# RaulAstudillo06/BOCF

Hardware: AMD Instinct MI355X
Metric: acquisition evals/sec (candidates x MC-samples/sec), uEI_noiseless batch call; GP-fit ms alongside (higher is better)
Workload: dtype f64; 1 GPU; BASELINE configs[2]: m=4 rbf-ARD GP, N=4096 d=8, S=1024 MC samples, C=65536 candidates, noise 1e-06, top-16 selection; N=4096, d=8, m=4, S=1024, C=65536, rccl_ranks_seen=0

## Files before the change

bocf_amd/_ffi.py:

```python
import contextlib
import ctypes
import os

import numpy as np

HERE = os.path.dirname(os.path.abspath(__file__))
LIB_PATH = os.path.join(HERE, "lib", "libbocf_hip.so")
PROBES_LIB_PATH = os.path.join(HERE, "lib", "libbocf_hip_probes.so")

KERN_RBF, KERN_SE, KERN_MATERN52, KERN_MATERN32 = 0, 1, 2, 3
ADD_NOISE, CLIP = 1, 2
ACQ_EI, ACQ_PI = 0, 1
UTIL_LINEAR, UTIL_NEG_SQ_DIST, UTIL_NEG_SUM_EXP, UTIL_NEG_EXP_COS, UTIL_ROSENBROCK = 0, 1, 2, 3, 4
UTIL_PROGRAM = 5
EU_MEAN, EU_CLOSED, EU_MC = 0, 1, 2
EU_MODES = {"mean": EU_MEAN, "closed": EU_CLOSED, "mc": EU_MC}


def eu_mode(mode):
    return EU_MODES[mode] if isinstance(mode, str) else int(mode)


_c_double_p = ctypes.POINTER(ctypes.c_double)
_c_ll_p = ctypes.POINTER(ctypes.c_longlong)
_ctx_p = ctypes.c_void_p

FDF_CALLBACK = ctypes.CFUNCTYPE(ctypes.c_int, ctypes.c_void_p, _c_double_p, ctypes.POINTER(ctypes.c_int), ctypes.c_int, ctypes.c_int, _c_double_p, _c_double_p)

SIGNATURES = {
    "bocf_version": (ctypes.c_int, []),
    "bocf_last_error": (ctypes.c_char_p, []),
    "bocf_create": (ctypes.c_int, [ctypes.c_int, ctypes.POINTER(_ctx_p)]),
    "bocf_destroy": (None, [_ctx_p]),
    "bocf_set_option": (ctypes.c_int, [_ctx_p, ctypes.c_char_p, ctypes.c_longlong]),
    "bocf_fit": (ctypes.c_int, [_ctx_p, _c_double_p, _c_double_p, ctypes.c_int, ctypes.c_int, ctypes.c_int, ctypes.c_int,
                                _c_double_p, _c_double_p, _c_double_p, ctypes.c_int, _c_double_p, _c_double_p]),
    "bocf_set_kernel_ids": (ctypes.c_int, [_ctx_p, ctypes.POINTER(ctypes.c_int), ctypes.c_int]),
    "bocf_update_targets": (ctypes.c_int, [_ctx_p, _c_double_p, _c_double_p]),
    "bocf_append": (ctypes.c_int, [_ctx_p, _c_double_p, _c_double_p, _c_double_p]),
    "bocf_lml_gradients": (ctypes.c_int, [_ctx_p, _c_double_p, _c_double_p, _c_double_p]),
    "bocf_infer": (ctypes.c_int, [_ctx_p, _c_double_p, _c_double_p, ctypes.c_int, ctypes.c_int, ctypes.c_int, ctypes.c_int, _c_double_p,
                                  _c_double_p, _c_double_p, ctypes.c_int, _c_double_p, _c_double_p, _c_double_p, _c_double_p, _c_double_p]),
    "bocf_last_fit_info": (ctypes.c_int, [_ctx_p, ctypes.POINTER(ctypes.c_int), ctypes.c_int]),
    "bocf_hmc": (ctypes.c_int, [_ctx_p, _c_double_p, _c_double_p, ctypes.c_int, ctypes.c_int, ctypes.c_int, ctypes.c_int, _c_double_p, ctypes.c_int,
                                ctypes.POINTER(ctypes.c_int), ctypes.c_double, ctypes.c_double, _c_double_p, _c_double_p, ctypes.c_int, ctypes.c_int,
                                ctypes.c_double, ctypes.c_int, ctypes.c_int, _c_double_p, ctypes.POINTER(ctypes.c_int), ctypes.POINTER(ctypes.c_int),
                                ctypes.POINTER(ctypes.c_int), _c_ll_p]),
    "bocf_hmc_streamed": (ctypes.c_int, [_ctx_p, _c_double_p, _c_double_p, ctypes.c_int, ctypes.c_int, ctypes.c_int, ctypes.c_int, _c_double_p, ctypes.c_int,
                                         ctypes.POINTER(ctypes.c_int), ctypes.c_double, ctypes.c_double, _c_double_p, _c_double_p, ctypes.c_int, ctypes.c_int,
                                         ctypes.c_double, _c_double_p, ctypes.POINTER(ctypes.c_int), ctypes.POINTER(ctypes.c_int),
                                         ctypes.POINTER(ctypes.c_int), _c_ll_p]),
    "bocf_get_factor": (ctypes.c_int, [_ctx_p, ctypes.c_int, _c_double_p, _c_double_p]),
    "bocf_get_train_kernel": (ctypes.c_int, [_ctx_p, ctypes.c_int, _c_double_p]),
    "bocf_set_posterior": (ctypes.c_int, [_ctx_p, ctypes.c_int, ctypes.c_int, ctypes.c_int, _c_double_p, _c_double_p, _c_double_p]),
    "bocf_set_candidates": (ctypes.c_int, [_ctx_p, _c_double_p, ctypes.c_int]),
    "bocf_predict": (ctypes.c_int, [_ctx_p, ctypes.c_int, _c_double_p, _c_double_p]),
    "bocf_predict_cov_column": (ctypes.c_int, [_ctx_p, ctypes.c_int, _c_double_p]),
    "bocf_predict_gradients": (ctypes.c_int, [_ctx_p, _c_double_p, _c_double_p]),
    "bocf_posterior_cov": (ctypes.c_int, [_ctx_p, _c_double_p, ctypes.c_int, _c_double_p, ctypes.c_int, ctypes.c_int, _c_double_p]),
    "bocf_posterior_samples": (ctypes.c_int, [_ctx_p, ctypes.c_int, _c_double_p, ctypes.c_int, ctypes.c_int, _c_double_p, _c_double_p]),
    "bocf_thompson_select": (ctypes.c_int, [_ctx_p, ctypes.c_int, _c_double_p, ctypes.c_int, _c_double_p, ctypes.c_int, ctypes.c_int, _c_ll_p,
                                            _c_double_p]),
    "bocf_set_ref_points": (ctypes.c_int, [_ctx_p, _c_double_p, ctypes.c_int]),
    "bocf_cov_to_ref": (ctypes.c_int, [_ctx_p, ctypes.c_int, _c_double_p, _c_double_p]),
    "bocf_conditioned_variance": (ctypes.c_int, [_ctx_p, ctypes.c_int, ctypes.c_int, _c_double_p, _c_double_p]),
    "bocf_acq_kg": (ctypes.c_int, [_ctx_p, ctypes.c_int, ctypes.c_int, _c_double_p, ctypes.c_int, _c_double_p, ctypes.c_int, _c_double_p, ctypes.c_int,
                                   _c_double_p, ctypes.c_int, _c_double_p, _c_double_p]),
# ... 133 lines not shown
```

bocf_amd/csrc/acq.hip:

```cpp
#include "bocf_internal.h"
#include <type_traits>
#include <cstdlib>
#include "../../include/bocf_hip.h"
#include "utility_dev.h"

__global__ __launch_bounds__(256) void best_so_far_kernel(const double* __restrict__ mu_train, int N, int m, int util_kind,
                                                          const double* __restrict__ theta, int theta_dim,
                                                          const double* __restrict__ params, double* __restrict__ best) {
  const int l = blockIdx.x;
  const double* th = theta + (long)l * theta_dim;
  double mx = -INFINITY;
  for (int i = threadIdx.x; i < N; i += 256) {
    double y[BOCF_MAX_M];
#pragma unroll
    for (int j = 0; j < BOCF_MAX_M; ++j) y[j] = j < m ? mu_train[(long)j * N + i] : 0.0;
    const double v = utility_eval(util_kind, th, params, y, m);
    mx = fmax(mx, v);
  }
  __shared__ double red[256];
  red[threadIdx.x] = mx;
  __syncthreads();
  for (int o = 128; o > 0; o >>= 1) {
    if (threadIdx.x < o) red[threadIdx.x] = fmax(red[threadIdx.x], red[threadIdx.x + o]);
    __syncthreads();
// ... 65 lines not shown
  double acq = 0.0;
  for (int l = 0; l < a.L; ++l) {
    const double* th = a.theta + (long)l * a.theta_dim;
    const double best = a.kind == BOCF_ACQ_EI ? a.best[l] : a.best[l] + 1e-6;
    double part = 0.0;
    for (int s = lane; s < a.S; s += 64) {
      double y[BOCF_MAX_M];
#pragma unroll
      for (int j = 0; j < BOCF_MAX_M; ++j) y[j] = j < a.m ? mu[j] + sg[j] * a.Wt[(long)j * a.S + s] : 0.0;
      const double v = utility_eval(a.util_kind, th, a.util_params, y, a.m);
      if (a.kind == BOCF_ACQ_EI) part += fmax(v - best, 0.0);
      else part += (v - best) > 0.0 ? 1.0 : 0.0;
    }
#pragma unroll
    for (int o = 32; o > 0; o >>= 1) part += __shfl_xor(part, o, 64);
    acq += (part / (double)a.S) * a.prob[l];
  }
  if (lane == 0) a.acq[c] = (a.accumulate ? a.acq[c] : 0.0) + acq * a.scale;
}

template <int M>
__global__ __launch_bounds__(256) void acq_mc_m_kernel(AcqArgs a) {
  const int lane = threadIdx.x & 63;
  const int c = blockIdx.x * 4 + (threadIdx.x >> 6);
  if (c >= a.C) return;
  double mu[M], sg[M];
#pragma unroll
  for (int j = 0; j < M; ++j) {
    mu[j] = a.mean[(long)j * a.ld + c];
    sg[j] = sqrt(a.var[(long)j * a.ld + c]);
  }
  double acq = 0.0;
  for (int l = 0; l < a.L; ++l) {
    const double* th = a.theta + (long)l * a.theta_dim;
    const double best = a.kind == BOCF_ACQ_EI ? a.best[l] : a.best[l] + 1e-6;
    double part = 0.0;
    for (int s = lane; s < a.S; s += 64) {
      double y[BOCF_MAX_M];
#pragma unroll
      for (int j = 0; j < BOCF_MAX_M; ++j) y[j] = 0.0;
#pragma unroll
      for (int j = 0; j < M; ++j) y[j] = mu[j] + sg[j] * a.Wt[(long)j * a.S + s];
      const double v = utility_eval(a.util_kind, th, a.util_params, y, M);
      if (a.kind == BOCF_ACQ_EI) part += fmax(v - best, 0.0);
      else part += (v - best) > 0.0 ? 1.0 : 0.0;
    }
#pragma unroll
    for (int o = 32; o > 0; o >>= 1) part += __shfl_xor(part, o, 64);
    acq += (part / (double)a.S) * a.prob[l];
  }
  if (lane == 0) a.acq[c] = (a.accumulate ? a.acq[c] : 0.0) + acq * a.scale;
}

void launch_acq_mc(const AcqArgs& a, hipStream_t s) {
  if (a.C == 0) return;
  if (a.util_kind == BOCF_UTIL_PROGRAM) {
    launch_acq_mc_prog(a, s);
    return;
  }
  const dim3 grid((unsigned)((a.C + 3) / 4));
  if (a.m >= 1 && a.m <= 8) {
#define LM(M) case M: BOCF_LAUNCH((acq_mc_m_kernel<M>), grid, dim3(256), 0, s, a); break;
    switch (a.m) { LM(1) LM(2) LM(3) LM(4) LM(5) LM(6) LM(7) LM(8) default: break; }
#undef LM
    return;
  }
  BOCF_LAUNCH(acq_mc_kernel, grid, dim3(256), 0, s, a);
}

__global__ __launch_bounds__(256) void acq_linear_grad_kernel(AcqArgs a) {
  const int c = blockIdx.x * 256 + threadIdx.x;
  if (c >= a.C) return;
  double mean[BOCF_MAX_M], var[BOCF_MAX_M];
#pragma unroll
  for (int j = 0; j < BOCF_MAX_M; ++j) {
    mean[j] = j < a.m ? a.mean[(long)j * a.ld + c] : 0.0;
    var[j] = j < a.m ? a.var[(long)j * a.ld + c] : 0.0;
  }
  double acq = 0.0;
  if (!a.accumulate)
    for (int q = 0; q < a.d; ++q) a.dacq[(long)c * a.d + q] = 0.0;
  for (int l = 0; l < a.L; ++l) {
    const double* th = a.theta + (long)l * a.theta_dim;
    double mu = 0.0, s2 = 0.0;
#pragma unroll
    for (int j = 0; j < BOCF_MAX_M; ++j)
      if (j < a.m) {
        mu += th[j] * mean[j];
        s2 += (th[j] * th[j]) * var[j];
      }
    const double sigma = sqrt(s2);
    double Phi, phi, u, val;
    if (a.kind == BOCF_ACQ_EI) {
      u = (mu - a.best[l]) / sigma;
      Phi = 0.5 * erfc(-u / 1.41421356237309504880);
      phi = exp(-0.5 * u * u) / 2.50662827463100050242;
      val = (mu - a.best[l]) * Phi + sigma * phi;
    } else {
      const double sfl = sigma < 1e-10 ? 1e-10 : sigma;
      u = (mu - (a.best[l] + 1e-6)) / sfl;
      Phi = 0.5 * erfc(-u / 1.41421356237309504880);
      phi = exp(-0.5 * u * u) / 2.50662827463100050242;
      val = Phi;
    }
    acq += val * a.prob[l];
    for (int q = 0; q < a.d; ++q) {
      double dmu = 0.0, dv = 0.0;
#pragma unroll
      for (int j = 0; j < BOCF_MAX_M; ++j)
        if (j < a.m) {
// ... 307 lines not shown
```

bocf_amd/csrc/bocf_ctx.h:

```cpp
#pragma once
#include "bocf_internal.h"
#include "chol_plan.h"
#include "predict_plan.h"
#include "../../include/bocf_hip.h"

#include <map>
#include <string>
#include <utility>
#include <vector>

int bocf_fail(const char* what, const char* detail);
void bocf_set_error(const char* text);
int bocf_launch_status();
int bocf_plan_cholesky(bocf_ctx* c, bool kinv, CholPlan* out);
int bocf_run_cholesky(bocf_ctx* c, const CholPlan& plan, bool counters_zeroed = false);
int bocf_run_trtri(bocf_ctx* c, bool early_done);
int bocf_comm_broadcast(bocf_ctx* c, double* buf, size_t count, int root);
int bocf_comm_group(bool start);
int bocf_comm_abort(bocf_ctx* c);
int bocf_comm_allreduce_sum(bocf_ctx* c, double* buf, size_t count);
#define fail bocf_fail
#define HIPCHK(expr)                                                         \
  do {                                                                       \
    hipError_t e_ = (expr);                                                  \
// ... 71 lines not shown
  long long fits_done = 0;
  int last_schedule = 0;
  int sched_m = 0;
  int force_sched_timeout = 0;
  int data_N = 0, data_d = 0, data_m = 0;
  int fused_infer = 1;
  int reuse_data = 0;
  int skip_mu_train = 0;
  DevBuf gpart, gout;
  DevBuf hmc_buf;
  double* infer_out = nullptr;
  size_t infer_out_cap = 0;
  bool fitted = false;
  bool canned = false;
  int N = 0, Np = 0, d = 0, m = 0, kernel_id = 0;
  long xs_stride = 0;
  std::vector<int> kernel_ids;
  std::vector<int> pending_ids;
  std::vector<KernHyp> hyp;
  std::vector<double> jitter;
  std::vector<int> last_info;
  DevBuf R32;
  bool r32_valid = false;
  int predict_f32 = 0;
  DevBuf Ri8, Ri8e, Ki8, Ki8e;
  bool ri8_valid = false;
  int predict_i8 = 0, i8_group = 0;
  DevBuf X, Xs, S, R, RT, E, ET, T, yc, tvec, rvec, dvec, alpha, lml, jit, hypd, info, mu_train;
  int C = 0;
  DevBuf Xc;
  long chunk = 65536;
  long workspace_mb = 24576;
  DevBuf Kstar, meanpart, sumsq, mean, var, acq, Vbuf, dmean, dvar, dacq, Vs, Ws;
  int pred_cap = 0;
  DevBuf theta, prob, best, params, Wt;
  std::vector<double> last_params;
  long long mu_epoch = 0;
  long long best_epoch = -1; int best_sig = -1;
  int S_mc = 0;
  bool have_acq = false;
  DevBuf prog_buf;
  UtilProg prog;
  DevBuf blk_idx, blk_val, out_idx, out_val;
  DevBuf eu_theta, eu_rows, eu_Z, eu_val, eu_grad;
  int eu_S = 0, eu_L = 0, eu_m = 0;
  void* eu_pin = nullptr;
  size_t eu_pin_cap = 0;
  hipEvent_t ev_eu_pin = nullptr;
  bool profile = false;
  double test_diag_shift = 0.0;
  int prefetch1 = 0;
  int kstar_valu_probe = 0;
  int small_path = 1;
  int hyper_samples = 1;
  int acq_hyper_samples = 0;
  int best_group = -1;
  int swizzle = -1;
  std::vector<std::pair<hipEvent_t, hipEvent_t>> events;
  double prof_flops = 0.0;
  std::map<std::string, std::vector<std::pair<hipEvent_t, hipEvent_t>>> phases;
  int shard_fit = 0;
  int shard_fit_simulate = 0;
  bool sharded = false;
  bocf_ctx* shard_helper = nullptr;
  DevBuf shard_meta;
  void* comm = nullptr;
  int world = 1, rank = 0;
  DevBuf pack, gidx, gval;
  bocf_ctx* ts_helper = nullptr;
  DevBuf ts_X, ts_K, ts_V, ts_mp, ts_mu, ts_Z, ts_jit, ts_u, ts_theta, ts_params, ts_out;
  std::vector<DevBuf> ts_F;
  std::vector<int> ts_S;
  int kg_na = 0;
  DevBuf kg_XA, kg_VA, kg_Wa, kg_muA, kg_s2A, kg_nug;
  DevBuf kg_V, kg_W, kg_cov, kg_s2c, kg_dcov, kg_dmean, kg_dvar, kg_par, kg_v0, kg_astar, kg_AB, kg_out, kg_dout;
};

int bocf_check_resident_program(bocf_ctx* c, const char* who, int m, int theta_dim, int n_util_params);
void bocf_thompson_drop(bocf_ctx* c);
void bocf_kg_drop(bocf_ctx* c);
int bocf_check_posterior(bocf_ctx* c, const char* who);
int bocf_group_range(bocf_ctx* c, const char* who, int group, int* j0, int* mg, int* per);
int bocf_enqueue_V(bocf_ctx* c, int j0, int mg, const double* Xq, int n, int npad, double* V, double* mu);


struct PhaseTimer {
  bocf_ctx* c;
  const char* name;
  hipEvent_t e0 = nullptr;
  PhaseTimer(bocf_ctx* ctx, const char* n) : c(ctx), name(n) {
    if (!c->profile) return;
    if (hipEventCreate(&e0) != hipSuccess) { e0 = nullptr; return; }
    (void)hipEventRecord(e0, c->stream);
  }
  void stop() {
    if (!e0) return;
    hipEvent_t e1 = nullptr;
    if (hipEventCreate(&e1) == hipSuccess) {
      (void)hipEventRecord(e1, c->stream);
      c->phases[name].emplace_back(e0, e1);
    } else {
      (void)hipEventDestroy(e0);
    }
    e0 = nullptr;
  }
  ~PhaseTimer() { stop(); }
// ... 21 lines not shown
```

bocf_amd/csrc/bocf_internal.h:

```cpp
#pragma once
#include <hip/hip_runtime.h>
#include <stdint.h>

#define BOCF_TILE 128
#define BOCF_MAX_D 32
#define BOCF_MAX_M 16
#define BOCF_MAX_FITS 1024
#define BOCF_MAX_L 32

void bocf_note_launch(const char* kernel, hipError_t e);
#define BOCF_LAUNCH(kern, grid, block, shm, stream, ...)              \
  do {                                                                \
    hipLaunchKernelGGL(kern, grid, block, shm, stream, __VA_ARGS__);  \
    bocf_note_launch(#kern, hipGetLastError());                       \
  } while (0)

__device__ __forceinline__ void dd_fma_acc(double& s, double& c, double a, double b) {
#pragma clang fp contract(off)
  const double p = a * b;
  const double e = __builtin_fma(a, b, -p);
  const double t = s + p;
  const double z = t - s;
  c += ((s - (t - z)) + (p - z)) + e;
  s = t;
// ... 171 lines not shown
                         double* mu_train, long ldmu, int m, hipStream_t s);

void launch_cross_kernel(const double* Xs, long strideXs, int N, int Np, int d, int kernel_id, const KernHyp* hyp,
                         const double* Xc, int c0, int Cn, int Cpad, const double* alpha, double* Kstar, long ldk, long strideK,
                         double* meanpart, double* meanlo, int nsplit, int m, int store_k, hipStream_t s, const int* kids = nullptr);
void launch_finalize_mean(const double* meanpart, const double* meanlo, int nsplit, int Cpad, const KernHyp* hyp, double* mean, long ldmean, int c0,
                          int Cn, int m, hipStream_t s);
void launch_finalize_var(const double* sumsq, int nrt, int Cpad, const KernHyp* hyp, int flags, double* var, long ldvar, int c0, int Cn, int m, hipStream_t s,
                         const double* meanpart = nullptr, const double* meanlo = nullptr, int nsplit = 0, double* mean = nullptr);
void launch_cov_column(const double* Xc, int C, int d, int kernel_id, const KernHyp* hyp, const double* t, long ldt, int flags, double* cov,
                       long ldcov, int m, hipStream_t s, const int* kids = nullptr);

#define BOCF_SMALL_N 16
void launch_gemv_small_t(const double* R, long strideR, int Np, const double* Kstar, long ldk, long strideK, double* V, int nc, int m, hipStream_t s);
void launch_sumsq_small(const double* V, int Np, double* sumsq, long ldo, int nc, int m, hipStream_t s);
void launch_gemv_small_n(const double* R, long strideR, int Np, const double* V, double* W, int nc, int m, hipStream_t s);
void launch_cross_small(const double* Xs, long strideXs, int N, int Np, int d, int kernel_id, const KernHyp* hyp, const double* Xc, int c0, int Cn, int nc,
                        const double* alpha, double* Kstar, long ldk, long strideK, double* meanpart, double* meanlo, int Cpad, int m, hipStream_t s,
                        const int* kids = nullptr);
void launch_gemv_small_t_mfma(const double* R, long strideR, int Np, const double* Kstar, long ldk, long strideK, double* V, double* sumsq, long ldss,
                              int nc, int m, hipStream_t s);
void launch_gemv_small_n_mfma(const double* RT, long strideR, int Np, const double* V, double* W, int nc, int m, hipStream_t s);

void launch_grad_kernel(const double* Xs, long strideXs, int N, int Np, int d, int kernel_id, const KernHyp* hyp, const double* Xc, int c0,
                        int Cn, const double* alpha, const double* W, long ldw, long strideW, double* dmean, double* dvar, long ldg,
                        int m, hipStream_t s, const int* kids = nullptr);

struct UtilProg {
  const unsigned* dev = nullptr;
  int m = 0, theta_dim = 0, n_slots = 0, n_val = 0, n_grad = 0, n_const = 0;
  int val_out = 0;
  int grad_out[1 + BOCF_MAX_M] = {0};
};
int util_prog_check(const char* who, const void* blob, long nbytes, int m, int theta_dim, UtilProg* out);
void util_prog_geometry(const UtilProg& p, int* threads, size_t* lds_bytes);

struct AcqArgs {
  const double* mean; const double* var; long ld;
  int m, C, L;
  int kind;
  int util_kind;
  int theta_dim;
  const double* theta;
  const double* prob;
  const double* best;
  const double* util_params; int n_util_params;
  const double* Wt; int S;
  double* acq;
  const double* dmean; const double* dvar; long ldg; int d;
  double* dacq;
  int accumulate;
  double scale;
  const UtilProg* prog;
};
void launch_best_so_far(const double* mu_train, int N, int m, int linear, int util_kind, const double* theta, int theta_dim, int L,
                        const double* util_params, double* best, hipStream_t s, const UtilProg* prog = nullptr);
void launch_acq_linear(const AcqArgs& a, hipStream_t s);
void launch_acq_mc(const AcqArgs& a, hipStream_t s);
void launch_acq_linear_grad(const AcqArgs& a, hipStream_t s);
void launch_acq_mc_grad(const AcqArgs& a, hipStream_t s);
struct EuArgs {
  const double* mean; const double* var; long ld;
  const double* dmean; const double* dvar; long ldg; int d;
  int m, C;
  int mode;
  int util_kind;
  int theta_dim;
  const double* theta;
  const int* rows;
  const double* util_params;
  const double* Zt; int S;
  double* val;
  double* grad;
  int accumulate;
  double scale;
  const UtilProg* prog;
};
void launch_eu(const EuArgs& a, hipStream_t s);
void launch_best_so_far_prog(const double* mu_train, int N, const double* theta, int theta_dim, int L, double* best, const UtilProg& p, hipStream_t s);
void launch_acq_mc_prog(const AcqArgs& a, hipStream_t s);
void launch_acq_mc_grad_prog(const AcqArgs& a, hipStream_t s);
void launch_eu_prog(const EuArgs& a, hipStream_t s);
void launch_thompson_util_prog(const double* F, int C, int S, const double* theta, int theta_dim, double* u, long ldu, const UtilProg& p, hipStream_t s);
void launch_topk(const double* acq, int C, int k, long long* blk_idx, double* blk_val, long long* out_idx, double* out_val, hipStream_t s);
int topk_num_blocks(int C);
void launch_pack_topk(const long long* idx, const double* val, int k, long long lo, int world, int rank, double* pack, hipStream_t s);
void launch_merge_packed(const double* pack, int k, int world, long long* gidx, double* gval, long long* out_idx, double* out_val, hipStream_t s);

void launch_post_cov(const double* V1, long ld1, long strideV1, const double* V2, long ld2, long strideV2, const double* X1, int n1, const double* X2,
                     int n2, int d, int K, int kernel_id, const int* kids, const KernHyp* hyp, const double* jitter, int sym, double* out, long ldo,
                     long strideO, int m, hipStream_t s);
void launch_post_diag(double* S, long ld, long strideS, int n, int mode, double* mean, const double* jit, int m, hipStream_t s);
void launch_post_sample(const double* U, long ldu, long strideU, const double* Z, const double* mu, long ldmu, int C, int S, double* F, int m,
                        hipStream_t s);
void launch_thompson_util(const double* F, int m, int C, int S, int util_kind, const double* theta, int theta_dim, const double* params, double* u,
                          long ldu, hipStream_t s, const UtilProg* prog = nullptr);

void launch_kg_diag(const double* V, long ldv, long strideV, int K, int n, const KernHyp* hyp, double* out, long ldo, int m, hipStream_t s);
void launch_cov_grad(const double* Xs, long strideXs, int N, int d, int kernel_id, const int* kids, const KernHyp* hyp, const double* Xc, int Cn,
                     const double* XA, int a0, int an, const double* Wa, long ldw, long strideW, double* out, int m, hipStream_t s);
void launch_cond_var(const double* cov, long ldc, long strideC, int q, const double* s2c, long lds, const double* s2A, long lda, const double* nug,
                     const double* ds2c, long ldg, const double* dcov, int C, int d, double* var, double* dvar, int m, hipStream_t s);
struct KgArgs {
  const double* cov; int ldc; long strideC;
  const double* s2c; int lds;
  const double* nug;
  const double* muA; const double* s2A; int lda;
  const double* v0;
  const double* Zf; int Sf;
  const double* theta; int theta_dim; const double* prob; int L;
  const double* util_params;
// ... 20 lines not shown
```

bocf_amd/csrc/capi.hip:

```cpp
#include "bocf_ctx.h"

#include <chrono>
#include <cmath>
#include <cstdio>
#include <cstdlib>
#include <cstring>
#include <string>
#include <vector>

static thread_local std::string g_err;
int bocf_fail(const char* what, const char* detail) {
  g_err = std::string(what) + ": " + (detail ? detail : "");
  return -1;
}
void bocf_set_error(const char* text) { g_err = text ? text : ""; }

static thread_local std::string g_launch_err;
void bocf_note_launch(const char* kernel, hipError_t e) {
  if (e != hipSuccess && g_launch_err.empty()) g_launch_err = std::string("launch of ") + kernel + ": " + hipGetErrorString(e);
}
int bocf_launch_status() {
  const hipError_t e = hipGetLastError();
  if (!g_launch_err.empty()) {
    g_err = g_launch_err;
// ... 85 lines not shown
  for (DevBuf* b : bufs) b->release();
  if (c->infer_out) (void)hipHostFree(c->infer_out);
  if (c->tile_ctr) (void)hipFree(c->tile_ctr);
  for (hipEvent_t ev : c->ev_chol) (void)hipEventDestroy(ev);
  for (hipStream_t st : {c->s_res, c->s_hi, c->s_bulk, c->s_inv})
    if (st) (void)hipStreamDestroy(st);
  if (c->ev_half) (void)hipEventDestroy(c->ev_half);
  if (c->ev_inv_early) (void)hipEventDestroy(c->ev_inv_early);
  (void)hipStreamDestroy(c->stream);
  delete c;
}

struct OptDesc {
  const char* name;
  long long lo, hi;
  int kind;
  void (*set)(bocf_ctx*, long long);
  bool (*extra)(long long);
  const char* what;
};
static bool opt_lookahead_ok(long long v) { return v == -1 || v == 0 || v == 2; }
#ifdef BOCF_PROBES
static bool opt_swizzle_ok(long long v) { return v == -1 || v == 0 || v == 1 || (v >= 100 && v < 164) || (v >= 256 && v <= 258); }
static bool opt_potrf_ok(long long v) { return v == 0 || (v >= 11 && v <= 14); }
#else
static bool opt_swizzle_ok(long long v) { return v == -1 || v == 0 || v == 258; }
#endif
static const OptDesc g_options[] = {
    {"chunk", 128, 1 << 24, 0, [](bocf_ctx* c, long long v) { c->chunk = (long)round_up((int)v, 128); }, nullptr, "candidates per pass (rounded up to 128)"},
    {"workspace_mb", 1, 1 << 20, 0, [](bocf_ctx* c, long long v) { c->workspace_mb = (long)v; }, nullptr, "cap of the per-pass K* workspace"},
    {"profile", 0, 1, 0, [](bocf_ctx* c, long long v) { c->profile = v != 0; }, nullptr, "HIP events around the dominant kernel and the named phases"},
    {"predict_f32", 0, 1, 1, [](bocf_ctx* c, long long v) { c->predict_f32 = v != 0; }, nullptr, "fp32 variance contraction (BASELINE configs[4])"},
    {"i8_group", 0, 64, 0, [](bocf_ctx* c, long long v) { c->i8_group = (int)v; }, nullptr, "predict_i8: 0 = workgroups in blocks of 4 row-tile pairs x 8 column tiles per XCD; g >= 1 = bands of g pairs x all column tiles"},
    {"predict_i8", 0, 1, 1, [](bocf_ctx* c, long long v) { c->predict_i8 = v != 0; }, nullptr, "variance contraction in exact int8 products (six radix-254 digits per operand column, fp64 recombination)"},
    {"fused_infer", 0, 1, 0, [](bocf_ctx* c, long long v) { c->fused_infer = v != 0; }, nullptr, "one fused launch per inference for N <= 128"},
    {"reuse_data", 0, 1, 1, [](bocf_ctx* c, long long v) { c->reuse_data = v != 0; }, nullptr, "next fits reuse the resident X / Y"},
    {"skip_mu_train", 0, 1, 1, [](bocf_ctx* c, long long v) { c->skip_mu_train = v != 0; }, nullptr, "do not refresh the mean at the training inputs"},
    {"aggregate", 0, 8, 0, [](bocf_ctx* c, long long v) { c->chol.aggregate = (int)v; }, nullptr, "panels per trailing update (0 = by size)"},
    {"lookahead", -1, 2, 0, [](bocf_ctx* c, long long v) { c->chol.lookahead = (int)v; }, opt_lookahead_ok,
     "factorization schedule: -1 by size, 0 single stream, 2 reserved-CU chain"},
    {"team_fit", -1, 1, 0, [](bocf_ctx* c, long long v) { c->chol.team_fit = (int)v; }, nullptr, "factorization + inverse in one launch by resident workgroup teams (-1 = by size)"},
    {"team_panels", 1, 32, 0, [](bocf_ctx* c, long long v) { c->chol.team_panels = (int)v; }, nullptr, "team schedule above 8 panels: panels per team launch (one trailing update each)"},
    {"team_hybrid", 0, 2, 0, [](bocf_ctx* c, long long v) { c->chol.team_hybrid = (int)v; }, nullptr, "more than 24 panels: launched schedule for the first block rows, one team launch for the rest"},
    {"team_tail_share", 1, 8, 0, [](bocf_ctx* c, long long v) { c->chol.team_tail_share = (int)v; }, nullptr, "hybrid schedule: eighths of the compute units the tail's teams take"},
    {"team_whole_max", 2, 32, 0, [](bocf_ctx* c, long long v) { c->chol.team_whole_max = (int)v; }, nullptr, "panels up to which one team launch does the whole factorization and inverse"},
    {"team_stream", 0, 1, 0, [](bocf_ctx* c, long long v) { c->chol.team_stream = (int)v; }, nullptr, "teams: the critical tiles are formed underneath the diagonal blocks, 16 rows at a time"},
    {"team_crit_load", 0, 4096, 0, [](bocf_ctx* c, long long v) { c->chol.team_crit_load = (int)v; }, nullptr, "teams: critical-chain workgroups carry nothing else while the others get by with <= this many units each"},
    {"lookahead_min_nb", 2, 1 << 20, 0, [](bocf_ctx* c, long long v) { c->chol.lookahead_min_nb = (int)v; }, nullptr, "reserved-CU schedule from this many panels"},
    {"merge_x3", 0, 2, 0, [](bocf_ctx* c, long long v) { c->chol.merge_x3 = (int)v; }, nullptr, "second product of an inverse merge in the three-buffer kernel"},
    {"shard_fit", 0, 1, 0, [](bocf_ctx* c, long long v) { c->shard_fit = v != 0; }, nullptr, "output-sharded fit over the communicator"},
    {"trsm_wave", 0, 1, 0, [](bocf_ctx* c, long long v) { c->chol.trsm_wave = v != 0; }, nullptr, "row solves through the wave-level single-tile kernel"},
    {"overlap_inverse", -1, 1, 0, [](bocf_ctx* c, long long v) { c->chol.overlap_inverse = (int)v; }, nullptr, "early part of the inverse underneath the factorization (-1 = by size)"},
    {"small_path", 0, 1, 0, [](bocf_ctx* c, long long v) { c->small_path = v != 0; }, nullptr, "GEMV-shaped path for <= 16 candidates"},
    {"prefetch1", 0, 1, 0, [](bocf_ctx* c, long long v) { c->prefetch1 = v != 0; }, nullptr, "one-tile-deep staging in the 128-row variance kernel"},
    {"swizzle", -1, 258, 0, [](bocf_ctx* c, long long v) { c->swizzle = (int)v; }, opt_swizzle_ok, "variance-GEMM tiling: -1 by size, 0 128-row tiles, 258 256-row tiles (probes build: also 1, 100..163, 256, 257)"},
    {"hyper_samples", 1, 64, 1,
     [](bocf_ctx* c, long long v) {
       if ((int)v != c->hyper_samples) c->S_mc = c->eu_S = 0;
       c->hyper_samples = (int)v;
     },
     nullptr, "the fitted outputs are H hyper-samples x m / H model outputs"},
    {"acq_hyper_samples", 0, 64, 1, [](bocf_ctx* c, long long v) { c->acq_hyper_samples = (int)v; }, nullptr, "hyper-samples the acquisitions average over (0 = all)"},
    {"best_group", -1, 63, 1, [](bocf_ctx* c, long long v) { c->best_group = (int)v; }, nullptr, "whose best-so-far every hyper-sample uses (-1 = its own)"},
#ifdef BOCF_PROBES
    {"potrf_scalar", 0, 14, 2, [](bocf_ctx* c, long long v) { c->chol.potrf_scalar = (int)v; }, opt_potrf_ok, "TIMING-ONLY variants of the diagonal-block kernel: 11..14 (wrong results)"},
    {"shard_fit_simulate", 0, 64, 2, [](bocf_ctx* c, long long v) { c->shard_fit_simulate = (int)v; }, nullptr, "TEST HOOK: one process plays all G ranks of a sharded fit"},
    {"kstar_valu_probe", 0, 4, 2, [](bocf_ctx* c, long long v) { c->kstar_valu_probe = (int)v; }, nullptr, "TIMING-ONLY variants of the two-buffer 256-row variance kernel (wrong results)"},
    {"test_diag_shift_1e12", -1000000000000000LL, 1000000000000000LL, 2, [](bocf_ctx* c, long long v) { c->test_diag_shift = (double)v * 1e-12; }, nullptr,
     "TEST HOOK: Ky diagonal -= value * 1e-12 (forces the jitter ladder)"},
    {"force_sched_timeout", 0, 1, 2, [](bocf_ctx* c, long long v) { c->force_sched_timeout = (int)v; }, nullptr, "TEST HOOK: the next gated schedule reports a dependency time-out"},
    {"force_cu_count", 0, 4096, 2, [](bocf_ctx* c, long long v) { c->chol.force_cu_count = (int)v; }, nullptr, "TEST HOOK: pretend the device has this many compute units (schedule selection)"},
#endif
};
static const int g_noptions = (int)(sizeof(g_options) / sizeof(g_options[0]));

static const OptDesc* find_option(const char* name) {
  for (int i = 0; i < g_noptions; ++i)
    if (!strcmp(name, g_options[i].name)) return &g_options[i];
  return nullptr;
}

extern "C" int bocf_option_count(void) { return g_noptions; }

extern "C" int bocf_option_info(int index, const char** name_out, long long* lo_out, long long* hi_out, int* kind_out, const char** what_out) {
  if (index < 0 || index >= g_noptions) return fail("bocf_option_info", "index out of range");
  const OptDesc& o = g_options[index];
  if (name_out) *name_out = o.name;
  if (lo_out) *lo_out = o.lo;
  if (hi_out) *hi_out = o.hi;
  if (kind_out) *kind_out = o.kind;
  if (what_out) *what_out = o.what;
  return 0;
}

extern "C" int bocf_option_check(const char* name, long long value) {
  if (!name) return fail("bocf_set_option", "null argument");
  const OptDesc* o = find_option(name);
  if (!o) return fail("bocf_set_option", (std::string("unknown option '") + name + "'").c_str());
  if (value < o->lo || value > o->hi || (o->extra && !o->extra(value)))
    return fail("bocf_set_option", (std::string(name) + " = " + std::to_string(value) + " is out of range: " + o->what).c_str());
  return 0;
}

extern "C" int bocf_set_option(bocf_ctx* c, const char* name, long long value) {
  if (!c || !name) return fail("bocf_set_option", "null argument");
  if (bocf_option_check(name, value)) return -1;
// ... 352 lines not shown
  c->last_params.swap(key);
  c->best_epoch = -1;
  return 0;
}

static int group_size(bocf_ctx* c, const char* where) {
  const int H = c->hyper_samples;
  if (c->m % H != 0) return fail(where, "the fitted outputs are not a multiple of option hyper_samples"), -1;
  if (c->best_group >= H) return fail(where, "option best_group is not a valid hyper-sample index"), -1;
  if (c->m / H > BOCF_MAX_M) return fail(where, "too many outputs per hyper-sample"), -1;
  return c->m / H;
}

static int copy_pair_out(bocf_ctx* c, const void* src0, double* out0, size_t b0, const void* src1, double* out1, size_t b1) {
  if (b0 + b1 > 0 && b0 + b1 <= BOCF_PIN_BYTES && pin_ensure(&c->pin_out, &c->pin_out_cap, b0 + b1) == 0) {
    char* pin = static_cast<char*>(c->pin_out);
    if (b0) HIPCHK(hipMemcpyAsync(pin, src0, b0, hipMemcpyDeviceToHost, c->stream));
    if (b1) HIPCHK(hipMemcpyAsync(pin + b0, src1, b1, hipMemcpyDeviceToHost, c->stream));
    HIPCHK(hipStreamSynchronize(c->stream));
    if (b0) memcpy(out0, pin, b0);
    if (b1) memcpy(out1, pin + b0, b1);
    LAUNCHCHK();
    return 0;
  }
  if (out1) HIPCHK(hipMemcpyAsync(out1, src1, b1, hipMemcpyDeviceToHost, c->stream));
  if (out0) HIPCHK(hipMemcpyAsync(out0, src0, b0, hipMemcpyDeviceToHost, c->stream));
  HIPCHK(hipStreamSynchronize(c->stream));
  LAUNCHCHK();
  return 0;
}

typedef void (*AcqLaunch)(const AcqArgs& a, hipStream_t s);

static void acq_over_hyper_samples(bocf_ctx* c, AcqArgs a, int m, int linear, AcqLaunch launch) {
  const int H = (c->acq_hyper_samples > 0 && c->acq_hyper_samples < c->hyper_samples) ? c->acq_hyper_samples : c->hyper_samples;
  const double* mean = a.mean; const double* var = a.var; const double* dmean = a.dmean; const double* dvar = a.dvar;
  for (int h = 0; h < H; ++h) {
    if (h == 0 || c->best_group < 0) {
      const int gb = c->best_group >= 0 ? c->best_group : h;
      const int sig = (linear ? 1 : 0) | (a.util_kind << 1) | (gb << 8);
      const bool cached = H == 1 && c->best_epoch == c->mu_epoch && c->best_sig == sig;
      c->best_epoch = H == 1 ? c->mu_epoch : -1;
      c->best_sig = sig;
      if (!cached)
      launch_best_so_far(c->mu_train.as<double>() + (size_t)gb * m * c->N, c->N, m, linear, a.util_kind, a.theta, a.theta_dim, a.L,
                         a.util_params, c->best.as<double>(), c->stream, a.prog);
    }
    a.mean = mean + (size_t)h * m * a.ld;
    a.var = var + (size_t)h * m * a.ld;
    if (dmean) { a.dmean = dmean + (size_t)h * m * a.ldg * a.d; a.dvar = dvar + (size_t)h * m * a.ldg * a.d; }
    a.accumulate = h > 0;
    a.scale = 1.0 / H;
    PhaseTimer t(c, "acq");
    launch(a, c->stream);
  }
}

static int run_acq(bocf_ctx* c, int m, bool linear, bool grad, AcqLaunch launch, int kind, int util_kind, const double* util_params, int n_util_params,
                   const double* theta, int theta_dim, const double* prob, int L, double* acq_out, double* dacq_out) {
  HIPCHK(hipSetDevice(c->device));
  if (c->C == 0) return 0;
  if (upload_acq_params(c, theta, theta_dim, prob, L, util_params, n_util_params)) return -1;
  if (run_predict(c, BOCF_ADD_NOISE | BOCF_CLIP, true, grad)) return -1;
  AcqArgs a{};
  a.mean = c->mean.as<double>(); a.var = c->var.as<double>(); a.ld = c->pred_cap;
  a.m = m; a.C = c->C; a.L = L; a.kind = kind; a.util_kind = util_kind; a.theta_dim = theta_dim > 0 ? theta_dim : 1;
  a.theta = c->theta.as<double>(); a.prob = c->prob.as<double>(); a.best = c->best.as<double>();
  a.util_params = c->params.as<double>(); a.n_util_params = n_util_params; a.acq = c->acq.as<double>();
  a.prog = &c->prog;
  if (!linear) { a.Wt = c->Wt.as<double>(); a.S = c->S_mc; }
  if (grad) { a.dmean = c->dmean.as<double>(); a.dvar = c->dvar.as<double>(); a.ldg = c->pred_cap; a.d = c->d; a.dacq = c->dacq.as<double>(); }
  acq_over_hyper_samples(c, a, m, linear ? 1 : 0, launch);
  c->have_acq = true;
  const size_t b0 = acq_out ? sizeof(double) * (size_t)c->C : 0, b1 = dacq_out ? sizeof(double) * (size_t)c->C * c->d : 0;
  return copy_pair_out(c, c->acq.p, acq_out, b0, c->dacq.p, dacq_out, b1);
}

extern "C" int bocf_acq_linear(bocf_ctx* c, int kind, const double* theta, const double* prob, int L, double* acq_out) {
  if (!c || !c->fitted) return fail("bocf_acq_linear", "model not fitted");
  if (kind != BOCF_ACQ_EI && kind != BOCF_ACQ_PI) return fail("bocf_acq_linear", "unknown acquisition kind");
  const int m = group_size(c, "bocf_acq_linear");
  if (m < 0) return -1;
  return run_acq(c, m, true, false, launch_acq_linear, kind, BOCF_UTIL_LINEAR, nullptr, 0, theta, m, prob, L, acq_out, nullptr);
}

extern "C" int bocf_acq_linear_grad(bocf_ctx* c, int kind, const double* theta, const double* prob, int L, double* acq_out,
                                    double* dacq_out) {
  if (!c || !c->fitted) return fail("bocf_acq_linear_grad", "model not fitted");
  if (kind != BOCF_ACQ_EI && kind != BOCF_ACQ_PI) return fail("bocf_acq_linear_grad", "unknown acquisition kind");
  const int m = group_size(c, "bocf_acq_linear_grad");
  if (m < 0) return -1;
  return run_acq(c, m, true, true, launch_acq_linear_grad, kind, BOCF_UTIL_LINEAR, nullptr, 0, theta, m, prob, L, acq_out, dacq_out);
}

extern "C" int bocf_set_mc_samples(bocf_ctx* c, const double* W, int S) {
  if (!c || !c->fitted || !W || S < 1) return fail("bocf_set_mc_samples", "model not fitted / bad samples");
  HIPCHK(hipSetDevice(c->device));
  const int m = group_size(c, "bocf_set_mc_samples");
  if (m < 0) return -1;
  std::vector<double> wt((size_t)m * S);
  for (int s = 0; s < S; ++s)
    for (int j = 0; j < m; ++j) wt[(long)j * S + s] = W[(long)s * m + j];
  if (c->Wt.ensure(sizeof(double) * wt.size())) return -1;
  HIPCHK(hipMemcpyAsync(c->Wt.p, wt.data(), sizeof(double) * wt.size(), hipMemcpyHostToDevice, c->stream));
  HIPCHK(hipStreamSynchronize(c->stream));
  c->S_mc = S;
  return 0;
}

static int mc_group_size(bocf_ctx* c, const char* me, int util_kind, const double* util_params, int n_util_params, int theta_dim) {
  if (util_kind < 0 || util_kind > BOCF_UTIL_PROGRAM) return fail(me, "unknown utility kind");
  if (c->S_mc < 1) return fail(me, "no Monte-Carlo samples set (bocf_set_mc_samples)");
  const int m = group_size(c, me);
  if (m < 0) return -1;
  if (util_kind == BOCF_UTIL_PROGRAM) return bocf_check_resident_program(c, me, m, theta_dim, n_util_params) ? -1 : m;
  if ((util_kind == BOCF_UTIL_LINEAR || util_kind == BOCF_UTIL_NEG_SQ_DIST) && theta_dim != m) return fail(me, "theta_dim must equal m");
  if (util_kind == BOCF_UTIL_ROSENBROCK && (theta_dim < 1 || (m & 1))) return fail(me, "rosenbrock utility needs theta_dim >= 1 and even m");
  if (util_kind == BOCF_UTIL_NEG_EXP_COS && n_util_params != m) return fail(me, "neg_exp_cos needs m weights");
  if (n_util_params > 0 && !util_params) return fail(me, "util_params is null");
  return m;
}

// ... 111 lines not shown
  return copy_pair_out(c, c->eu_val.p, val_out, sizeof(double) * (size_t)C, c->eu_grad.p, grad_out, need_grad ? sizeof(double) * (size_t)C * d : 0);
}

extern "C" int bocf_select_topk(bocf_ctx* c, int k, long long* idx_out, double* val_out) {
  if (!c || !c->have_acq) return fail("bocf_select_topk", "no acquisition vector on the device");
  if (k < 1 || k > 64 || !idx_out) return fail("bocf_select_topk", "k out of range (1..64) / null out");
  HIPCHK(hipSetDevice(c->device));
  const int nb = topk_num_blocks(c->C);
  if (c->blk_idx.ensure(sizeof(long long) * (size_t)nb * k) || c->blk_val.ensure(sizeof(double) * (size_t)nb * k) ||
      c->out_idx.ensure(8 * (size_t)128))
    return -1;
  {
    PhaseTimer t(c, "topk");
    launch_topk(c->acq.as<double>(), c->C, k, c->blk_idx.as<long long>(), c->blk_val.as<double>(), c->out_idx.as<long long>(),
                reinterpret_cast<double*>(c->out_idx.as<long long>() + k), c->stream);
  }
  long long host[128];
  HIPCHK(hipMemcpyAsync(host, c->out_idx.p, 8 * (size_t)(val_out ? 2 * k : k), hipMemcpyDeviceToHost, c->stream));
  HIPCHK(hipStreamSynchronize(c->stream));
  memcpy(idx_out, host, sizeof(long long) * k);
  if (val_out) memcpy(val_out, host + k, sizeof(double) * k);
  LAUNCHCHK();
  return 0;
}

extern "C" int bocf_profile_read(bocf_ctx* c, double* ms_out, long long* launches_out, double* flops_out, int reset) {
  if (!c) return fail("bocf_profile_read", "null ctx");
  HIPCHK(hipSetDevice(c->device));
  HIPCHK(hipStreamSynchronize(c->stream));
  double ms = 0.0;
  for (auto& pr : c->events) {
    float t = 0.f;
    HIPCHK(hipEventElapsedTime(&t, pr.first, pr.second));
    ms += t;
  }
  if (ms_out) *ms_out = ms;
  if (launches_out) *launches_out = (long long)c->events.size();
  if (flops_out) *flops_out = c->prof_flops;
  if (reset) {
    drop_events(c);
    c->prof_flops = 0.0;
  }
  return 0;
}

extern "C" int bocf_get_stat(bocf_ctx* c, const char* name, long long* value_out) {
  if (!c || !name || !value_out) return fail("bocf_get_stat", "null argument");
  if (!strcmp(name, "sched_timeouts")) *value_out = c->sched_timeouts;
  else if (!strcmp(name, "gated_schedules_off")) *value_out = c->gated_off;
  else if (!strcmp(name, "last_schedule")) *value_out = c->last_schedule;
  else if (!strcmp(name, "early_inverse")) *value_out = c->early_inverse_started;
  else if (!strcmp(name, "cu_masks_ok")) *value_out = c->cu_masks_ok;
  else if (!strcmp(name, "comm_world")) *value_out = c->comm ? c->world : 0;
  else if (!strcmp(name, "kstar_workspace_bytes")) *value_out = (long long)c->Kstar.cap;
  else return fail("bocf_get_stat", "unknown statistic");
  return 0;
}

extern "C" int bocf_profile_phase(bocf_ctx* c, const char* name, double* ms_out, long long* count_out, int reset) {
  if (!c || !name) return fail("bocf_profile_phase", "null argument");
  HIPCHK(hipSetDevice(c->device));
  HIPCHK(hipStreamSynchronize(c->stream));
  double ms = 0.0;
  long long n = 0;
  auto it = c->phases.find(name);
  if (it != c->phases.end()) {
    for (auto& pr : it->second) {
      float t = 0.f;
      HIPCHK(hipEventElapsedTime(&t, pr.first, pr.second));
      ms += t;
      ++n;
    }
    if (reset) {
      for (auto& pr : it->second) {
        (void)hipEventDestroy(pr.first);
        (void)hipEventDestroy(pr.second);
      }
      c->phases.erase(it);
    }
  }
  if (ms_out) *ms_out = ms;
  if (count_out) *count_out = n;
  return 0;
}
```

include/bocf_hip.h:

```cpp
#ifndef BOCF_HIP_H
#define BOCF_HIP_H

#ifdef __cplusplus
extern "C" {
#endif

typedef struct bocf_ctx bocf_ctx;

enum { BOCF_KERN_RBF = 0, BOCF_KERN_SE = 1, BOCF_KERN_MATERN52 = 2, BOCF_KERN_MATERN32 = 3 };

enum { BOCF_ADD_NOISE = 1,
       BOCF_CLIP = 2 };

enum { BOCF_ACQ_EI = 0,
       BOCF_ACQ_PI = 1 };

enum { BOCF_UTIL_LINEAR = 0, BOCF_UTIL_NEG_SQ_DIST = 1, BOCF_UTIL_NEG_SUM_EXP = 2,
       BOCF_UTIL_NEG_EXP_COS = 3, BOCF_UTIL_ROSENBROCK = 4,
       BOCF_UTIL_PROGRAM = 5 };

#define BOCF_PROG_MAGIC 0x47505542u
#define BOCF_PROG_VERSION 1
#define BOCF_PROG_HEADER_WORDS 32
#define BOCF_PROG_MAX_INSTR 1024
#define BOCF_PROG_MAX_SLOTS 64
#define BOCF_PROG_MAX_CONSTS 256
enum { BOCF_OP_ADD = 0, BOCF_OP_SUB, BOCF_OP_MUL, BOCF_OP_DIV, BOCF_OP_NEG, BOCF_OP_ABS, BOCF_OP_SIGN, BOCF_OP_SQRT, BOCF_OP_EXP, BOCF_OP_LOG,
       BOCF_OP_SIN, BOCF_OP_COS, BOCF_OP_TANH, BOCF_OP_POW, BOCF_OP_MIN, BOCF_OP_MAX,
       BOCF_OP_GE,
       BOCF_OP_COUNT };
enum { BOCF_OPERAND_SLOT = 0, BOCF_OPERAND_INPUT = 1, BOCF_OPERAND_PARAM = 2, BOCF_OPERAND_CONST = 3 };

int bocf_version(void);
const char* bocf_last_error(void);

int bocf_create(int device, bocf_ctx** out);
void bocf_destroy(bocf_ctx* ctx);

int bocf_set_option(bocf_ctx* ctx, const char* name, long long value);

int bocf_fit(bocf_ctx* ctx, const double* X, const double* Y, int N, int d, int m, int kernel_id,
             const double* variance, const double* lengthscale, const double* noise,
             int max_jitter_tries, double* jitter_out, double* lml_out);

int bocf_set_kernel_ids(bocf_ctx* ctx, const int* ids, int m);

int bocf_update_targets(bocf_ctx* ctx, const double* Y, double* lml_out);

int bocf_append(bocf_ctx* ctx, const double* x_new, const double* Y, double* lml_out);

int bocf_lml_gradients(bocf_ctx* ctx, double* dvariance_out, double* dlengthscale_out, double* dnoise_out);

int bocf_infer(bocf_ctx* ctx, const double* X, const double* Y, int N, int d, int m, int kernel_id, const double* variance,
               const double* lengthscale, const double* noise, int max_jitter_tries, double* jitter_out, double* lml_out,
               double* dvariance_out, double* dlengthscale_out, double* dnoise_out);

int bocf_hmc(bocf_ctx* ctx, const double* X, const double* Y, int N, int d, int m, int kernel_id, double* theta, int nls, const int* fixed,
             double prior_a, double prior_b, const double* momenta, const double* uniforms, int num_samples, int hmc_iters, double stepsize,
             int max_jitter_tries, int raise_on_failure, double* chains_out, int* accepted_out, int* diverged_out, int* status_out,
             long long* inferences_out);

int bocf_hmc_streamed(bocf_ctx* ctx, const double* X, const double* Y, int N, int d, int m, int kernel_id, double* theta, int nls,
                      const int* fixed, double prior_a, double prior_b, const double* momenta, const double* uniforms, int num_samples,
                      int hmc_iters, double stepsize, double* chains_out, int* accepted_out, int* diverged_out, int* draws_done_out,
                      long long* inferences_out);

int bocf_last_fit_info(bocf_ctx* ctx, int* info_out, int n);

int bocf_get_factor(bocf_ctx* ctx, int j, double* L_out, double* alpha_out);
int bocf_get_train_kernel(bocf_ctx* ctx, int j, double* K_out);

int bocf_set_posterior(bocf_ctx* ctx, int m, int C, int N, const double* mean, const double* var, const double* mu_train);

int bocf_set_candidates(bocf_ctx* ctx, const double* Xc, int C);

int bocf_predict(bocf_ctx* ctx, int flags, double* mean_out, double* var_out);

int bocf_predict_cov_column(bocf_ctx* ctx, int flags, double* cov0_out);

int bocf_posterior_cov(bocf_ctx* ctx, const double* X1, int n1, const double* X2, int n2, int group, double* cov_out);
int bocf_posterior_samples(bocf_ctx* ctx, int group, const double* Z, int S, int max_jitter_tries, double* samples_out, double* jitter_out);
int bocf_thompson_select(bocf_ctx* ctx, int util_kind, const double* util_params, int n_util_params, const double* theta, int theta_dim, int k,
                         long long* idx_out, double* val_out);

int bocf_predict_gradients(bocf_ctx* ctx, double* dmean_out, double* dvar_out);

int bocf_mean_at_train(bocf_ctx* ctx, double* out);

int bocf_acq_linear(bocf_ctx* ctx, int kind, const double* theta, const double* prob, int L, double* acq_out);

int bocf_acq_linear_grad(bocf_ctx* ctx, int kind, const double* theta, const double* prob, int L, double* acq_out, double* dacq_out);
// ... 60 lines not shown
```

Before: 1.098 billion evals/s.

## Add register-resident MC acquisition kernel with persistent waves over candidate runs

Adds a Monte-Carlo acquisition kernel that keeps the normal samples in registers for the whole wave and has each wave walk a contiguous run of candidates. Each candidate's mean and variance are prefetched one step ahead. The grid is sized to the CU count times waves per SIMD. This removes the repeated global reloads of the sample matrix per candidate that the old one-wave-per-candidate kernel paid. The cost is high register pressure (M*NI doubles) and less parallelism. It applies only to linear and negative-squared-distance utilities and is enabled by default for C at or above 4096.

Measured after the change: 1.099 billion evals/s (median of 6 runs). No clear change (+0.1%).

```diff
diff --git a/bocf_amd/_ffi.py b/bocf_amd/_ffi.py
--- a/bocf_amd/_ffi.py
+++ b/bocf_amd/_ffi.py
@@ -13,6 +13,7 @@
 ACQ_EI, ACQ_PI = 0, 1
 UTIL_LINEAR, UTIL_NEG_SQ_DIST, UTIL_NEG_SUM_EXP, UTIL_NEG_EXP_COS, UTIL_ROSENBROCK = 0, 1, 2, 3, 4
 UTIL_PROGRAM = 5
+ACQ_RESIDENT_MIN_C = 4096
 EU_MEAN, EU_CLOSED, EU_MC = 0, 1, 2
 EU_MODES = {"mean": EU_MEAN, "closed": EU_CLOSED, "mc": EU_MC}
 
diff --git a/bocf_amd/csrc/acq.hip b/bocf_amd/csrc/acq.hip
--- a/bocf_amd/csrc/acq.hip
+++ b/bocf_amd/csrc/acq.hip
@@ -141,10 +141,138 @@
   if (lane == 0) a.acq[c] = (a.accumulate ? a.acq[c] : 0.0) + acq * a.scale;
 }
 
+constexpr int ACQ_RESIDENT_MAX_SLOTS = 64;
+constexpr int ACQ_RESIDENT_WAVES_PER_SIMD = 2;
+template <int M, int NI, int KIND>
+__device__ __forceinline__ void acq_mc_resident_run(const AcqArgs& a, const int lane, const int c0, const int c1) {
+  double w[M][NI];
+#pragma unroll
+  for (int j = 0; j < M; ++j)
+#pragma unroll
+    for (int i = 0; i < NI; ++i) w[j][i] = lane + 64 * i < a.S ? a.Wt[(long)j * a.S + lane + 64 * i] : 0.0;
+  double mn[M], vr[M];
+#pragma unroll
+  for (int j = 0; j < M; ++j) {
+    mn[j] = a.mean[(long)j * a.ld + c0];
+    vr[j] = a.var[(long)j * a.ld + c0];
+  }
+  for (int c = c0; c < c1; ++c) {
+    double mu[M], sg[M];
+#pragma unroll
+    for (int j = 0; j < M; ++j) {
+      mu[j] = mn[j];
+      sg[j] = sqrt(vr[j]);
+    }
+    constexpr bool AHEAD = M * NI + 5 * M <= 100;
+    const int cn = c + 1 < c1 ? c + 1 : c;
+    auto fetch_next = [&]() {
+#pragma unroll
+      for (int j = 0; j < M; ++j) {
+        mn[j] = a.mean[(long)j * a.ld + cn];
+        vr[j] = a.var[(long)j * a.ld + cn];
+      }
+    };
+    if (AHEAD) fetch_next();
+    double acq = 0.0;
+    for (int l = 0; l < a.L; ++l) {
+      double th[BOCF_MAX_M];
+#pragma unroll
+      for (int j = 0; j < BOCF_MAX_M; ++j) th[j] = j < M ? a.theta[(long)l * a.theta_dim + j] : 0.0;
+      const double best = a.kind == BOCF_ACQ_EI ? a.best[l] : a.best[l] + 1e-6;
+      double sl[M];
+#pragma unroll
+      for (int j = 0; j < M; ++j) {
+        sl[j] = sg[j];
+        asm volatile("" : "+v"(sl[j]));
+      }
+      auto sweep = [&](auto ei) {
+        constexpr bool EI = decltype(ei)::value;
+        constexpr int G = NI < 4 ? NI : 4;
+        double part = 0.0;
+#pragma unroll
+        for (int g = 0; g < NI; g += G) {
+          if (64 * g < a.S) {
+#pragma unroll
+            for (int i = g; i < g + G; ++i) {
+              double y[BOCF_MAX_M];
+#pragma unroll
+              for (int j = 0; j < BOCF_MAX_M; ++j) y[j] = 0.0;
+#pragma unroll
+              for (int j = 0; j < M; ++j) y[j] = mu[j] + sl[j] * w[j][i];
+              double v = utility_eval(KIND, th, a.util_params, y, M);
+              asm("" : "+v"(v));
+              const double sum = EI ? part + fmax(v - best, 0.0) : part + ((v - best) > 0.0 ? 1.0 : 0.0);
+              part = lane + 64 * i < a.S ? sum : part;
+            }
+          }
+        }
+        return part;
+      };
+      double part = a.kind == BOCF_ACQ_EI ? sweep(std::true_type()) : sweep(std::false_type());
+#pragma unroll
+      for (int o = 32; o > 0; o >>= 1) part += __shfl_xor(part, o, 64);
+      acq += (part / (double)a.S) * a.prob[l];
+    }
+    if (lane == 0) a.acq[c] = (a.accumulate ? a.acq[c] : 0.0) + acq * a.scale;
+    if (!AHEAD) fetch_next();
+  }
+}
+
+template <int M, int NI>
+__global__ __launch_bounds__(256, 2) void acq_mc_resident_kernel(AcqArgs a, int run) {
+  const int lane = threadIdx.x & 63;
+  const int wave = blockIdx.x * 4 + __builtin_amdgcn_readfirstlane(threadIdx.x >> 6);
+  const long lo = (long)wave * run;
+  if (lo >= a.C) return;
+  const int c0 = (int)lo, c1 = (int)(lo + run < a.C ? lo + run : a.C);
+  if (a.util_kind == BOCF_UTIL_LINEAR) acq_mc_resident_run<M, NI, BOCF_UTIL_LINEAR>(a, lane, c0, c1);
+  else acq_mc_resident_run<M, NI, BOCF_UTIL_NEG_SQ_DIST>(a, lane, c0, c1);
+}
+
+template <int M, int NI>
+static void launch_acq_mc_resident_mn(const AcqArgs& a, dim3 grid, int run, hipStream_t s) {
+  if constexpr (M * NI <= ACQ_RESIDENT_MAX_SLOTS) BOCF_LAUNCH((acq_mc_resident_kernel<M, NI>), grid, dim3(256), 0, s, a, run);
+}
+
+template <int M>
+static void launch_acq_mc_resident_m(const AcqArgs& a, int ni, dim3 grid, int run, hipStream_t s) {
+  switch (ni) {
+    case 1: launch_acq_mc_resident_mn<M, 1>(a, grid, run, s); break;
+    case 2: launch_acq_mc_resident_mn<M, 2>(a, grid, run, s); break;
+    case 4: launch_acq_mc_resident_mn<M, 4>(a, grid, run, s); break;
+    case 8: launch_acq_mc_resident_mn<M, 8>(a, grid, run, s); break;
+    default: launch_acq_mc_resident_mn<M, 16>(a, grid, run, s); break;
+  }
+}
+
+int acq_mc_resident_slots(const AcqArgs& a) {
+  if (a.util_kind == BOCF_UTIL_PROGRAM || a.C == 0) return 0;
+  if (a.resident == 0 || a.ncu < 1 || a.m < 1 || a.m > 8 || a.S < 1) return 0;
+  if (a.util_kind != BOCF_UTIL_LINEAR && a.util_kind != BOCF_UTIL_NEG_SQ_DIST) return 0;
+  if (a.resident == 1 && a.C < BOCF_ACQ_RESIDENT_MIN_C) return 0;
+  const int need = (a.S + 63) / 64;
+  if ((long)a.m * need > ACQ_RESIDENT_MAX_SLOTS) return 0;
+  int ni = 1;
+  while (ni < need) ni *= 2;
+  if (ni > 16 || a.m * ni > ACQ_RESIDENT_MAX_SLOTS) return 0;
+  return ni;
+}
+
 void launch_acq_mc(const AcqArgs& a, hipStream_t s) {
   if (a.C == 0) return;
   if (a.util_kind == BOCF_UTIL_PROGRAM) {
     launch_acq_mc_prog(a, s);
+    return;
+  }
+  if (const int ni = acq_mc_resident_slots(a)) {
+    const int wps = a.resident >= 2 ? a.resident : ACQ_RESIDENT_WAVES_PER_SIMD;
+    const long waves = (long)a.ncu * 4 * wps;
+    const int run = (int)((a.C + waves - 1) / waves);
+    const long used = ((long)a.C + run - 1) / run;
+    const dim3 rgrid((unsigned)((used + 3) / 4));
+#define LM(M) case M: launch_acq_mc_resident_m<M>(a, ni, rgrid, run, s); break;
+    switch (a.m) { LM(1) LM(2) LM(3) LM(4) LM(5) LM(6) LM(7) LM(8) default: break; }
+#undef LM
     return;
   }
   const dim3 grid((unsigned)((a.C + 3) / 4));
diff --git a/bocf_amd/csrc/bocf_ctx.h b/bocf_amd/csrc/bocf_ctx.h
--- a/bocf_amd/csrc/bocf_ctx.h
+++ b/bocf_amd/csrc/bocf_ctx.h
@@ -147,6 +147,8 @@
   int prefetch1 = 0;
   int kstar_valu_probe = 0;
   int small_path = 1;
+  int acq_resident = 1;
+  long long acq_resident_launches = 0;
   int hyper_samples = 1;
   int acq_hyper_samples = 0;
   int best_group = -1;
diff --git a/bocf_amd/csrc/bocf_internal.h b/bocf_amd/csrc/bocf_internal.h
--- a/bocf_amd/csrc/bocf_internal.h
+++ b/bocf_amd/csrc/bocf_internal.h
@@ -247,11 +247,14 @@
   int accumulate;
   double scale;
   const UtilProg* prog;
+  int resident;
+  int ncu;
 };
 void launch_best_so_far(const double* mu_train, int N, int m, int linear, int util_kind, const double* theta, int theta_dim, int L,
                         const double* util_params, double* best, hipStream_t s, const UtilProg* prog = nullptr);
 void launch_acq_linear(const AcqArgs& a, hipStream_t s);
 void launch_acq_mc(const AcqArgs& a, hipStream_t s);
+int acq_mc_resident_slots(const AcqArgs& a);
 void launch_acq_linear_grad(const AcqArgs& a, hipStream_t s);
 void launch_acq_mc_grad(const AcqArgs& a, hipStream_t s);
 struct EuArgs {
diff --git a/bocf_amd/csrc/capi.hip b/bocf_amd/csrc/capi.hip
--- a/bocf_amd/csrc/capi.hip
+++ b/bocf_amd/csrc/capi.hip
@@ -161,6 +161,7 @@
     {"trsm_wave", 0, 1, 0, [](bocf_ctx* c, long long v) { c->chol.trsm_wave = v != 0; }, nullptr, "row solves through the wave-level single-tile kernel"},
     {"overlap_inverse", -1, 1, 0, [](bocf_ctx* c, long long v) { c->chol.overlap_inverse = (int)v; }, nullptr, "early part of the inverse underneath the factorization (-1 = by size)"},
     {"small_path", 0, 1, 0, [](bocf_ctx* c, long long v) { c->small_path = v != 0; }, nullptr, "GEMV-shaped path for <= 16 candidates"},
+    {"acq_resident", 0, 4, 0, [](bocf_ctx* c, long long v) { c->acq_resident = (int)v; }, nullptr, "Monte-Carlo acquisition with the normals in registers and a wave per run of candidates: 0 never, 1 from BOCF_ACQ_RESIDENT_MIN_C candidates, 2..4 always, with that many waves per SIMD"},
     {"prefetch1", 0, 1, 0, [](bocf_ctx* c, long long v) { c->prefetch1 = v != 0; }, nullptr, "one-tile-deep staging in the 128-row variance kernel"},
     {"swizzle", -1, 258, 0, [](bocf_ctx* c, long long v) { c->swizzle = (int)v; }, opt_swizzle_ok, "variance-GEMM tiling: -1 by size, 0 128-row tiles, 258 256-row tiles (probes build: also 1, 100..163, 256, 257)"},
     {"hyper_samples", 1, 64, 1,
@@ -619,6 +620,7 @@
     a.accumulate = h > 0;
     a.scale = 1.0 / H;
     PhaseTimer t(c, "acq");
+    if (launch == launch_acq_mc && acq_mc_resident_slots(a)) c->acq_resident_launches++;
     launch(a, c->stream);
   }
 }
@@ -635,6 +637,7 @@
   a.theta = c->theta.as<double>(); a.prob = c->prob.as<double>(); a.best = c->best.as<double>();
   a.util_params = c->params.as<double>(); a.n_util_params = n_util_params; a.acq = c->acq.as<double>();
   a.prog = &c->prog;
+  a.resident = c->acq_resident; a.ncu = c->ncu;
   if (!linear) { a.Wt = c->Wt.as<double>(); a.S = c->S_mc; }
   if (grad) { a.dmean = c->dmean.as<double>(); a.dvar = c->dvar.as<double>(); a.ldg = c->pred_cap; a.d = c->d; a.dacq = c->dacq.as<double>(); }
   acq_over_hyper_samples(c, a, m, linear ? 1 : 0, launch);
@@ -852,6 +855,7 @@
   else if (!strcmp(name, "early_inverse")) *value_out = c->early_inverse_started;
   else if (!strcmp(name, "cu_masks_ok")) *value_out = c->cu_masks_ok;
   else if (!strcmp(name, "comm_world")) *value_out = c->comm ? c->world : 0;
+  else if (!strcmp(name, "acq_resident_launches")) *value_out = c->acq_resident_launches;
   else if (!strcmp(name, "kstar_workspace_bytes")) *value_out = (long long)c->Kstar.cap;
   else return fail("bocf_get_stat", "unknown statistic");
   return 0;
diff --git a/include/bocf_hip.h b/include/bocf_hip.h
--- a/include/bocf_hip.h
+++ b/include/bocf_hip.h
@@ -37,6 +37,7 @@
 int bocf_create(int device, bocf_ctx** out);
 void bocf_destroy(bocf_ctx* ctx);
 
+#define BOCF_ACQ_RESIDENT_MIN_C 4096
 int bocf_set_option(bocf_ctx* ctx, const char* name, long long value);
 
 int bocf_fit(bocf_ctx* ctx, const double* X, const double* Y, int N, int d, int m, int kernel_id,
```
